# Dellintel98/smart-nanogrid-gym

Measured on AMD Instinct MI355X. Metric: env-steps/sec (whole node) at N=65,536 envs × 10 chargers, 24-step day, higher is better.
Workload: dtype f64; 1 GPU; 65536 envs/GPU x 10 chargers x 24-step day, b-pv bounded sparse 1h, GPU-RNG reset + 24 fused steps per bench step (hipGraph); envs_per_gpu=65536, chargers=10, step_unit=one simulated day of every env, days_per_graph_replay=11, parallelism=env-sharded x1

## Files before the change

include/sng.h:

```cpp
#ifndef SNG_H
#define SNG_H

#include <stddef.h>
#include <stdint.h>

#ifdef __cplusplus
extern "C" {
#endif

#define SNG_ABI_VERSION 10

typedef enum SngStatus {
    SNG_OK = 0,
    SNG_ERR_INVALID_ARGUMENT = -1,
    SNG_ERR_UNSUPPORTED = -2,
    SNG_ERR_HIP = -3,
    SNG_ERR_STATE = -4,
    SNG_ERR_OUT_OF_MEMORY = -5
} SngStatus;

typedef enum SngPenaltyMode {
    SNG_PENALTY_NONE = 0,
    SNG_PENALTY_ON_DEPARTURE = 1,
    SNG_PENALTY_SPARSE = 2,
// ... 130 lines not shown

int sng_state_size(const SngEnv *env, int with_episode_return, size_t *bytes);
int sng_get_state(SngEnv *env, void *host_buf, size_t bytes, const double *episode_return, void *stream);
int sng_set_state(SngEnv *env, const void *host_buf, size_t bytes, double *episode_return, void *stream);

int sng_get_scenario(SngEnv *env, int64_t first, int64_t count, int32_t max_vehicles, double *soc,
                     double *occupancy, double *capacity, double *requested_soc, int32_t *arrivals,
                     int32_t *departures, int32_t *n_vehicles, double *pv_ratio, void *stream);

int sng_get_tables(const SngEnv *env, double *irr, double *irr_max, double *pv_power, double *price,
                   double *price_max, int32_t *n);

#define SNG_GRAPH_RESET 1
#define SNG_GRAPH_STEP_NODES 2
#define SNG_GRAPH_TRAJECTORY 4
int sng_graph_create(SngEnv *env, const float *actions, float *obs, double *reward, uint8_t *done,
                     const SngInfo *info, int flags, int32_t days, double *day_returns, SngGraph **out);
int sng_graph_launch(SngGraph *graph, void *stream);
int sng_graph_step_nodes(const SngGraph *graph);
int sng_time_step_kernels(SngEnv *env, const float *actions, float *obs, double *reward, uint8_t *done,
                          const SngInfo *info, int32_t days, float *ms, float *reset_ms, void *stream);
void sng_graph_destroy(SngGraph *graph);

int sng_host_generate_scenarios(const SngConfig *cfg, int64_t num_envs, uint64_t seed, int32_t episodes,
                                double *soc, double *occupancy, double *capacity, double *requested_soc,
                                int32_t *arrivals, int32_t *departures, int32_t max_vehicles,
                                double *pv_ratio);

int32_t sng_host_threads(void);

int sng_get_day_counter(SngEnv *env, uint64_t *out, void *stream);

int sng_bandwidth_probe(int device, int64_t read_bytes, int64_t write_bytes, int32_t reps, float *dispatch_us,
                        float *back_to_back_us, void *stream);
// ... 15 lines not shown
```

smart-nanogrid-gym_amd/csrc/sng_api.cpp:

```cpp
#include <atomic>
#include <condition_variable>
#include <cstring>
#include <mutex>
#include <thread>

#include "sng_env.h"
#include "sng_host_day.h"
#include "sng_host_pool.h"
#include "sng_mt.h"

using namespace sng;

namespace sng {

thread_local std::string g_create_error;

int ensure_req(SngEnv *env) {
    if (!env->ds.req) HIP_TRY(env, hipMalloc(&env->ds.req, env->timeline() * sizeof(double)));
    return SNG_OK;
}

int await_prepare(SngEnv *env, hipStream_t st) {
    if (env->prep_launched) HIP_TRY(env, hipStreamWaitEvent(st, env->prep_done, 0));
    return SNG_OK;
}

int alloc_streams(SngEnv *env, RefStreams &r) {
    if (r.mt) return SNG_OK;
    HIP_TRY(env, hipMalloc(&r.mt, (size_t)env->E * 2 * kMtN * sizeof(uint32_t)));
    HIP_TRY(env, hipMalloc(&r.pos, (size_t)env->E * sizeof(int32_t)));
    return SNG_OK;
}

// ... 294 lines not shown
    *out = env;
    return SNG_OK;
}

void sng_destroy(SngEnv *env) {
    if (!env) return;
    DeviceScope scope(env->device);
    if (env->prep_stream) {
        (void)hipStreamSynchronize(env->prep_stream);
        (void)hipStreamDestroy(env->prep_stream);
        (void)hipEventDestroy(env->prep_done);
        (void)hipEventDestroy(env->day_drawn);
    }
    DeviceState &ds = env->ds;
    void *dev[] = {ds.soc, ds.bess, ds.bess0, ds.ratio, ds.pen0, ds.word, ds.aux, ds.req, ds.flags, ds.prof_key,
                   ds.episode, env->d_tables, env->rs.mt, env->rs.pos, env->ps.mt, env->ps.pos};
    for (void *x : dev)
        if (x) (void)hipFree(x);
    void *host[] = {env->h_word, env->h_aux, env->h_req, env->h_ratio, env->h_pen0};
    for (void *x : host)
        if (x) (void)hipHostFree(x);
    if (env->staging_done) (void)hipEventDestroy(env->staging_done);
    if (env->hio) (void)hipHostFree(env->hio);
    delete env;
}

int sng_get_dims(const SngEnv *env, SngDims *out) {
    if (!env || !out) return SNG_ERR_INVALID_ARGUMENT;
    out->obs_dim = env->p.obs_dim;
    out->act_dim = env->p.act_dim;
    out->timesteps = env->p.T;
// ... 383 lines not shown
```

smart-nanogrid-gym_amd/csrc/sng_env.h:

```cpp
#pragma once
#include <hip/hip_runtime.h>

#include <string>
#include <vector>

#include "sng.h"
#include "sng_device_scope.h"
#include "sng_host_tables.h"
#include "sng_launch.h"
#include "sng_layout.h"
#include "sng_state_format.h"

struct SngEnv {
    SngConfig cfg{};
    sng::Params p{};
    sng::HostTables tables;
    sng::Tables host_tab{};
    uint64_t cfg_hash = 0;
    std::vector<double> irradiance;
    int device = 0;
    int64_t E = 0;
    uint64_t seed = 0;
    int t = -1;
    bool day_finished = false;
    sng::DaySpans spans{0, 0, 0, sng::kSlots};
    int gen_mode = -1;
    bool gen_loaded = false;
    uint64_t replays = 0;
    sng::DeviceState ds{};
    sng::Tables *d_tables = nullptr;
    uint32_t *h_word = nullptr;
    double *h_aux = nullptr, *h_req = nullptr, *h_ratio = nullptr, *h_pen0 = nullptr;
    hipEvent_t staging_done = nullptr;
    sng::RefStreams rs{};
    bool np_seeded = false;
    hipStream_t prep_stream = nullptr;
    hipEvent_t prep_done = nullptr, day_drawn = nullptr;
    bool prep_launched = false;

    bool prepared = false;
    sng::RefStreams ps{};
    bool py_seeded = false;
    char *hio = nullptr, *hio_dev = nullptr;
    size_t hio_bytes = 0;
    std::string err;

    size_t timeline() const { return (size_t)p.T * p.n * (size_t)E; }
};

struct SngGraph {
    SngEnv *env = nullptr;
    bool with_reset = false;
    bool day_kernel = false;
    sng::DayKey key{};
    uint64_t seed = 0;
    int64_t env_offset = 0;
    hipGraph_t graph = nullptr;
    hipGraphExec_t exec = nullptr;
};

#pragma GCC visibility push(hidden)
namespace sng {

extern thread_local std::string g_create_error;

inline int fail(SngEnv *env, int code, const std::string &msg) {
    if (env) env->err = msg; else g_create_error = msg;
    return code;
// ... 53 lines not shown
    o.bess_power = i->battery_power_value;
    o.bess_calc_power = i->battery_calculated_power;
    o.nonexistent = i->nonexistent_vehicle_penalty;
    o.bess_initial = i->initial_battery_soc;
    o.flags = i->flags;
    o.episode_return = i->episode_return;
    o.charger_power = i->charger_power;
    o.vehicle_soc = i->vehicle_soc;
    o.flag_any = i->flag_summary;
    return o;
}

inline hipStream_t as_stream(void *s) { return (hipStream_t)s; }

int ensure_req(SngEnv *env);
int await_prepare(SngEnv *env, hipStream_t st);
int alloc_streams(SngEnv *env, RefStreams &r);
int ensure_np_streams(SngEnv *env, hipStream_t st);

}
#pragma GCC visibility pop
```

smart-nanogrid-gym_amd/csrc/sng_generate.h:

```cpp
#pragma once

namespace sng {

struct HashStream {
    uint32_t key, ctr;
    __device__ __forceinline__ uint32_t next() { return mix32(key + (ctr++) * 0x9e3779b9u); }
};

__device__ __forceinline__ double u32_unit(uint32_t x) { return (double)x * 0x1.0p-32; }

__device__ __forceinline__ int below(uint32_t x, int n) {
    return (int)(((uint64_t)x * (uint64_t)n) >> 32);
}

constexpr uint32_t kDomainRatio = 0x7a710000u;
constexpr uint32_t kDomainReplay = 0x7a720000u;

__device__ __forceinline__ double pv_ratio_draw(uint64_t seed, uint64_t ge, uint64_t day) {
    HashStream r2{stream_key(seed, ge, kDomainRatio, day), 0u};
    return (double)below(r2.next(), 181) / 100;
}

__device__ __forceinline__ double replay_ratio_draw(uint64_t seed, uint64_t ge, uint64_t replay) {
    HashStream r2{stream_key(seed, ge, kDomainReplay, replay), 0u};
// ... 167 lines not shown
    const uint32_t r = ((x1 & 0xffu) << 8) | (x2 & 0xffu);
    const uint32_t rc = r * 105u;
    d.cap = p.diff_caps ? 15u + (rc >> 16) : 40u;
    const uint32_t yd = (p.diff_caps ? rc : r) & 0xffffu;
    const int hi_c = d.ta + i10, hi_d = p.T + i1;
    const int high = hi_c < hi_d ? hi_c : hi_d;
    const int low = d.ta + i4;
    d.dep = (low >= high) ? low : low + (int)(__umul24(yd, (uint32_t)(high - low)) >> 16);
    d.req_draw = p.req_enabled ? rng.next() : 0u;
    return d;
}

constexpr int kObsParts = kGenBlock / kWave;
constexpr int kObsEnvs = kGenBlock / kObsParts;
constexpr int kObsBlocks = kGenBlock / kObsEnvs;
__device__ __forceinline__ void observe_day0(const Params &p, const DeviceState &s, uint64_t seed, int64_t E, int i4,
                                             int i10, int i1, uint64_t day, float *__restrict__ obs,
                                             double *__restrict__ ep_return, int vec_io, float *lds, int q) {
    const int n = p.n, O = p.obs_dim;
    const int tid = threadIdx.x, part = __builtin_amdgcn_readfirstlane(tid / kWave), le = tid % kWave;
    const int64_t e0 = (int64_t)blockIdx.x * kGenBlock + (int64_t)q * kObsEnvs;
    if (e0 >= E) return;
    const int nblk = (int)((E - e0) < kObsEnvs ? (E - e0) : kObsEnvs);
    const int64_t e = e0 + le;
    float *o_row = lds + le * O;
    if (le < nblk) {
        const uint64_t ge = (uint64_t)(e + p.env_offset);
        const uint64_t env_seed = p.seed + (uint64_t)p.env_offset + (uint64_t)e;
        if (p.noise && part == 0) {
            s.prof_key[2 * e] = stream_key(env_seed, 0, kDomainPV, day);
            s.prof_key[2 * e + 1] = stream_key(env_seed, 0, kDomainPrice, day);
        }
        if (part == 0) {
            const double ratio = pv_ratio_draw(seed, ge, day);
            s.ratio[e] = ratio;
            s.pen0[e] = 0.0;
            double fpv[4] = {1.0, 1.0, 1.0, 1.0}, fpr[4] = {1.0, 1.0, 1.0, 1.0};
            if (p.noise) {
#pragma unroll
                for (int k = 0; k < 4; ++k) {
                    if (p.pv_noise != 0.0) fpv[k] = profile_factor(env_seed, kDomainPV, day, k, p.pv_noise);
                    if (p.price_noise != 0.0) fpr[k] = profile_factor(env_seed, kDomainPrice, day, k, p.price_noise);
                }
            }
            write_obs_header(o_row, p, s.tables->irr_norm, s.tables->price_norm, ratio, fpv, fpr);
            if (p.bess) o_row[O - 1] = (float)s.bess[e];
            if (ep_return) ep_return[e] = 0.0;
        }
        const int k = p.pv ? 8 : 4;
        const uint32_t el8 = (uint32_t)e * 8u;
        for (int c0 = 2 * (part - 1); part > 0 && c0 < n; c0 += 2 * (kObsParts - 1)) {
            double soc0[2] = {0.0, 0.0};
#pragma unroll
            for (int i = 0; i < 2; ++i) {
                const int c = c0 + i;
                if (c >= n) break;
                GenStream rng{gen_key(seed, ge, (uint32_t)c, day), 0u};
                const VehicleDraw d = draw_vehicle(p, rng, 0, i4, i10, i1);
                const bool occ0 = d.ta == 0;
                soc0[i] = occ0 ? d.soc : 0.0;
                o_row[k + c] = (float)soc0[i];
                o_row[k + n + c] = departure_obs(pack_word(occ0, occ0, false, 0u, occ0 ? (uint32_t)d.dep : 0u));
            }
            const SocOff so = soc_off(c0, n, E, el8);
            if (c0 + 1 < n)
                bst2<kNT>(s.soc, so.v, soc0[0], soc0[1], so.s);
            else
                bst<kNT>(s.soc, so.v, soc0[0], so.s);
        }
    }
    __syncthreads();
    copy_out<kGenBlock>(obs + e0 * O, lds, nblk * O, vec_io != 0, tid);
}

constexpr int kGenRecPol = kNT;
__host__ __device__ constexpr int gen_part_lanes(int w) { return w == 3 ? 4 : w; }
__host__ __device__ constexpr int gen_rows(int n) { return 4 * (n / 4) + (n % 4 == 0 ? 0 : 4 * gen_part_lanes(n % 4) / 4); }
constexpr int kVehArrShift = 24;
constexpr uint32_t kVehRecMask = 0x3fff8u;
template <int TT, bool REQ>
__global__ __launch_bounds__(kGenBlock) void generate_kernel(Params p, DeviceState s, uint64_t seed, int64_t E,
                                                             int i4, int i10, int i1, float *__restrict__ obs,
                                                             double *__restrict__ ep_return, int vec_io) {
    extern __shared__ __attribute__((aligned(16))) float lds[];
    uint32_t *s_veh = reinterpret_cast<uint32_t *>(lds);
    uint32_t *s_car = s_veh + kDaySlots * kGenBlock;
    double *s_req = reinterpret_cast<double *>(s_car + kDaySlots * kGenBlock);
    const int tid = threadIdx.x;
    const int u = (int)blockIdx.y;
    const uint64_t day = *s.episode;
    if (u >= gen_rows(p.n)) {
        observe_day0(p, s, seed, E, i4, i10, i1, day, obs, ep_return, vec_io, lds, u - gen_rows(p.n));
        return;
    }
    const int full = 4 * (p.n / 4);
    const int q4 = u < full ? (u >> 2) * 4 : p.n & ~3;
    const int qw = p.n - q4 < 4 ? p.n - q4 : 4;
    const int lpe = u < full ? 4 : gen_part_lanes(qw);
    const int sub = u < full ? (u & 3) : u - full;
    const int c = q4 + tid % lpe;
    const int64_t e = (int64_t)blockIdx.x * kGenBlock + (int64_t)sub * (kGenBlock / lpe) + tid / lpe;
    if (e >= E || c >= p.n) return;
    const uint64_t ge = (uint64_t)(e + p.env_offset);
    GenStream rng{gen_key(seed, ge, (uint32_t)c, day), 0u};
    const int T = TT > 0 ? TT : p.T;
// ... 71 lines not shown
```

smart-nanogrid-gym_amd/csrc/sng_graph.cpp:

```cpp
#include <algorithm>

#include "sng_env.h"

using namespace sng;

extern "C" {

int sng_graph_create(SngEnv *env, const float *actions, float *obs, double *reward, uint8_t *done,
                     const SngInfo *info, int flags, int32_t days, double *day_returns, SngGraph **out) {
    const bool with_reset = (flags & SNG_GRAPH_RESET) != 0;
    if (!env || !actions || !obs || !reward || !done || !out) return fail(env, SNG_ERR_INVALID_ARGUMENT, "null argument");
    if (days < 1 || (days > 1 && !with_reset))
        return fail(env, SNG_ERR_INVALID_ARGUMENT, "days must be >= 1 (more than one needs SNG_GRAPH_RESET)");
    if (with_reset && !device_rng_ok(env))
        return fail(env, SNG_ERR_UNSUPPORTED, "device RNG needs time_interval <= 2h");
    ON_DEVICE_OF(env);
    if (env->p.req_enabled) SNG_TRY(ensure_req(env));
    hipStream_t cs;
    HIP_TRY(env, hipStreamCreateWithFlags(&cs, hipStreamNonBlocking));
    SngGraph *g = new SngGraph();
    g->env = env;
    g->with_reset = with_reset;
    g->key = with_reset ? DayKey::device_day(env->p) : DayKey::of(env->p);
    const Params p = with_day(env->p, g->key);
    g->seed = env->seed;
    g->env_offset = p.env_offset;
    const InfoPtrs ip = info_ptrs(info);
    const DaySpans &sp = env->spans;
    const int64_t E = env->E;
    const int A = p.act_dim;
    const int vec = (aligned16(actions) && aligned16(obs)) ? 1 : 0;
    const bool traj = (flags & SNG_GRAPH_TRAJECTORY) != 0;
    const size_t obs_block = (size_t)E * (size_t)p.obs_dim;
    const int64_t obs_step = traj ? (int64_t)obs_block : 0, out_step = traj ? E : 0;
    g->day_kernel = !(flags & SNG_GRAPH_STEP_NODES) && day_kernel_available(p, ip, traj) != 0;
    hipError_t e = hipStreamBeginCapture(cs, hipStreamCaptureModeThreadLocal);
    for (int d = 0; e == hipSuccess && d < days; ++d) {
        InfoPtrs ipd = ip;
        if (day_returns) ipd.episode_return = day_returns + (size_t)d * E;
        float *obs0 = obs + (traj ? (size_t)d * (size_t)(p.T + 1) * obs_block : 0);
        float *obs_d = obs0 + obs_step;
        double *reward_d = reward + (traj ? (size_t)d * (size_t)p.T * (size_t)E : 0);
        uint8_t *done_d = done + (traj ? (size_t)d * (size_t)p.T * (size_t)E : 0);
        if (with_reset) {
            e = launch_generate(p, env->ds, env->seed, E, sp.i4, sp.i10, sp.i1, obs0, ipd.episode_return,
                                (vec && aligned16(obs0)) ? 1 : 0, cs);
        }
        if (g->day_kernel) {
            if (e == hipSuccess)
                e = launch_day(p, env->ds, ipd, actions, obs_d, reward_d, done_d, E, 0, p.T,
                               (vec && aligned16(obs_d)) ? 1 : 0, cs, obs_step, out_step);
            continue;
        }
        for (int t = 0; e == hipSuccess && t < p.T; ++t) {
            float *obs_t = obs_d + (size_t)t * (size_t)obs_step;
            e = launch_step(p, env->ds, ipd, env->host_tab, actions + (size_t)t * E * A, obs_t,
                            reward_d + (size_t)t * (size_t)out_step, done_d + (size_t)t * (size_t)out_step, E, t,
                            (vec && aligned16(obs_t)) ? 1 : 0, cs);
        }
    }
    hipGraph_t graph = nullptr;
    hipError_t e2 = hipStreamEndCapture(cs, &graph);
    if (e == hipSuccess) e = e2;
    if (e == hipSuccess) e = hipGraphInstantiate(&g->exec, graph, nullptr, nullptr, 0);
    (void)hipStreamDestroy(cs);
    if (e != hipSuccess) {
        if (graph) (void)hipGraphDestroy(graph);
        delete g;
        return hip_fail(env, e, "graph capture");
    }
    g->graph = graph;
    *out = g;
    return SNG_OK;
}

int sng_graph_launch(SngGraph *g, void *stream) {
    if (!g) return SNG_ERR_INVALID_ARGUMENT;
    SngEnv *env = g->env;
    if (!g->with_reset) {
        if (!(g->key == DayKey::of(env->p)))
// ... 6 lines not shown
        return fail(env, SNG_ERR_STATE, "seed or env offset changed since the graph was captured: recapture it");
    ON_DEVICE_OF(env);
    if (g->with_reset) HIP_TRY(env, count_unstepped_device_day(env, as_stream(stream)));
    HIP_TRY(env, hipGraphLaunch(g->exec, as_stream(stream)));
    if (g->with_reset) {
        load_day(env, g->key);
        generated_day_loaded(env, SNG_RNG_DEVICE);
    }
    days_ran(env);
    return SNG_OK;
}

int sng_graph_step_nodes(const SngGraph *g) {
    if (!g) return -1;
    return g->day_kernel ? 1 : g->env->p.T;
}

void sng_graph_destroy(SngGraph *g) {
    if (!g) return;
    DeviceScope scope(g->env->device);
    if (g->exec) (void)hipGraphExecDestroy(g->exec);
    if (g->graph) (void)hipGraphDestroy(g->graph);
    delete g;
}

int sng_time_step_kernels(SngEnv *env, const float *actions, float *obs, double *reward, uint8_t *done,
                          const SngInfo *info, int32_t days, float *ms, float *reset_ms, void *stream) {
    if (!env || !actions || !obs || !reward || !done || days < 1)
        return fail(env, SNG_ERR_INVALID_ARGUMENT, "null argument");
    if (!device_rng_ok(env)) return fail(env, SNG_ERR_UNSUPPORTED, "device RNG needs time_interval <= 2h");
// ... 79 lines not shown
```

smart-nanogrid-gym_amd/csrc/sng_kernels.hip:

```cpp
#include <hip/hip_ext.h>
#include <hip/hip_runtime.h>
#include <stdint.h>

#include "sng.h"
#include "sng_launch.h"
#include "sng_layout.h"
#include "sng_step_plan.h"

#include "sng_dev_util.h"
#include "sng_dev_sums.h"
#include "sng_dev_env.h"
#include "sng_step_lean.h"
#include "sng_step_wide.h"
#include "sng_step_day.h"
#include "sng_step_general.h"
#include "sng_generate.h"

namespace sng {

__global__ __launch_bounds__(256) void probe_copy_kernel(const float4 *__restrict__ in, float4 *__restrict__ out,
                                                         int64_t nr, int64_t nw) {
    const int64_t i = (int64_t)blockIdx.x * 256 + threadIdx.x;
    typedef float v4f __attribute__((ext_vector_type(4)));
    v4f v = {0.f, 0.f, 0.f, 0.f};
// ... 146 lines not shown
    else return nullptr;
}
template <int NC>
static StepLaunch day_lean_launch(const StepPlan &pl, int64_t E, DayLeanKernel &kern) {
    kern = day_lean_entry<NC, false, false>();
    if (pl.pk && pl.req) kern = day_lean_entry<NC, true, true>();
    else if (pl.pk) kern = day_lean_entry<NC, true, false>();
    else if (pl.req) kern = day_lean_entry<NC, false, true>();
    return {nullptr, nullptr, blocks_for(E, kLeanBlock), dim3(kLeanBlock), LeanLds<NC>::BYTES};
}

int day_kernel_available(const Params &p, const InfoPtrs &info, bool trajectory) {
    return day_kernel_of(step_plan(p, info_diag(info)), trajectory) != DAY_NONE ? 1 : 0;
}

hipError_t launch_day(const Params &p, const DeviceState &s, const InfoPtrs &info, const float *act, float *obs,
                      double *reward, uint8_t *done, int64_t E, int t0, int nt, int vec_io, hipStream_t stream,
                      int64_t obs_step, int64_t out_step) {
    const StepPlan pl = step_plan(p, info_diag(info));
    const DayFamily fam = day_kernel_of(pl, obs_step != 0 || out_step != 0);
    if (fam == DAY_NONE) return hipErrorNotSupported;
    if (t0 < 0 || nt < 1 || t0 + nt > p.T) return hipErrorInvalidValue;
    if (fam == DAY_WIDE) {
        DayKernel kern = nullptr;
        const StepLaunch l = day_launch<10>(pl, E, kern);
        return launch_kernel(kern, l.grid, l.block, l.lds, stream, nullptr, nullptr, act, obs, reward, done, E, t0, nt,
                             vec_io, p, s, info);
    }
    DayLeanKernel kern = nullptr;
    StepLaunch l;
// ... 18 lines not shown
hipError_t launch_observe0(const Params &p, const DeviceState &s, float *obs, double *ep_return, int64_t E,
                           int vec_io, hipStream_t stream, int mode, int64_t replay, const RefStreams *ps, int py) {
    const RefStreams no_streams{nullptr, nullptr};
    const RefStreams &pss = (py && ps) ? *ps : no_streams;
    if (!ps) py = 0;
    const bool big = (size_t)round4(256 * p.obs_dim) * 4 <= 64 * 1024;
    const int envs = big ? 256 : kWave;
    auto kern = big ? (p.packed ? observe0_kernel<256, true> : observe0_kernel<256, false>)
                    : (p.packed ? observe0_kernel<kWave, true> : observe0_kernel<kWave, false>);
    return launch_kernel(kern, blocks_for(E, envs), dim3(envs), (size_t)round4(envs * p.obs_dim) * 4, stream, nullptr,
                         nullptr, p, s, obs, ep_return, E, vec_io, mode, replay, pss, py);
}

hipError_t launch_generate(const Params &p, const DeviceState &s, uint64_t seed, int64_t E, int i4, int i10, int i1,
                           float *obs, double *ep_return, int vec_io, hipStream_t stream, hipEvent_t ev_start,
                           hipEvent_t ev_stop) {
    const size_t veh = generate_lds_bytes(p.req_enabled != 0), tile = (size_t)round4(kObsEnvs * p.obs_dim) * 4;
    const bool fused = tile <= 32 * 1024;
    const dim3 grid((unsigned)((E + kGenBlock - 1) / kGenBlock), (unsigned)(gen_rows(p.n) + (fused ? kObsBlocks : 0))),
        block(kGenBlock);
    const size_t lds = (fused && tile > veh) ? tile : veh;
    const bool req = p.req_enabled != 0;
    auto kern = p.T == 24 ? (req ? generate_kernel<24, true> : generate_kernel<24, false>)
                : (p.T == 96 && !req) ? generate_kernel<96, false>
                : (req ? generate_kernel<0, true> : generate_kernel<0, false>);
    if (fused && ev_start && ev_stop)
        return launch_kernel(kern, grid, block, lds, stream, ev_start, ev_stop, p, s, seed, E, i4, i10, i1, obs,
                             ep_return, vec_io);
    if (ev_start) (void)hipEventRecord(ev_start, stream);
    hipError_t e = launch_kernel(kern, grid, block, lds, stream, nullptr, nullptr, p, s, seed, E, i4, i10, i1, obs,
                                 ep_return, vec_io);
    if (!fused) {
        if (e == hipSuccess) e = launch_profiles(p, s, E, stream);
        if (e == hipSuccess) e = launch_observe0(p, s, obs, ep_return, E, vec_io, stream, OBS0_DEVICE, -1);
    }
    if (e == hipSuccess && ev_stop) e = hipEventRecord(ev_stop, stream);
    return e;
}

}

#include "sng_ref_day.h"

namespace sng {

static int ref_day2_envs(int64_t E) {
// ... 40 lines not shown
    if (prepare) {
        hipError_t e = launch_mt_prepare(rs, E, stream);
        if (e != hipSuccess) return e;
    }
    const bool req = p.req_stream != 0;
    if (p.T == 24) {
        if (req) launch_ref_day2<24, true>(p, s, rs, E, i4, i10, i1, stream);
        else launch_ref_day2<24, false>(p, s, rs, E, i4, i10, i1, stream);
    } else {
        if (req) launch_ref_day2<0, true>(p, s, rs, E, i4, i10, i1, stream);
        else launch_ref_day2<0, false>(p, s, rs, E, i4, i10, i1, stream);
    }
    return hipGetLastError();
}

__global__ void bump_day_kernel(DeviceState s) { *s.episode += 1; }

hipError_t launch_bump_day(const DeviceState &s, hipStream_t stream) {
    hipLaunchKernelGGL(bump_day_kernel, dim3(1), dim3(1), 0, stream, s);
    return hipGetLastError();
}

hipError_t launch_profiles(const Params &p, const DeviceState &s, int64_t E, hipStream_t stream) {
    if (!p.noise) return hipSuccess;
    const dim3 grid((unsigned)((E + 255) / 256)), block(256);
    hipLaunchKernelGGL(profile_kernel, grid, block, 0, stream, p, s, E);
    return hipGetLastError();
}

}
```

smart-nanogrid-gym_amd/csrc/sng_launch.h:

```cpp
#pragma once
#include <hip/hip_runtime.h>

#include "sng_layout.h"

namespace sng {

hipError_t launch_step(const Params &p, const DeviceState &s, const InfoPtrs &info, const Tables &tab,
                       const float *act, float *obs, double *reward, uint8_t *done, int64_t E, int t, int vec_io,
                       hipStream_t stream, hipEvent_t ev_start = nullptr, hipEvent_t ev_stop = nullptr);
int day_kernel_available(const Params &p, const InfoPtrs &info, bool trajectory = false);
hipError_t launch_day(const Params &p, const DeviceState &s, const InfoPtrs &info, const float *act, float *obs,
                      double *reward, uint8_t *done, int64_t E, int t0, int nt, int vec_io, hipStream_t stream,
                      int64_t obs_step = 0, int64_t out_step = 0);
hipError_t launch_observe0(const Params &p, const DeviceState &s, float *obs, double *ep_return, int64_t E,
                           int vec_io, hipStream_t stream, int mode, int64_t replay, const RefStreams *ps = nullptr,
                           int py = 0);
hipError_t launch_generate(const Params &p, const DeviceState &s, uint64_t seed, int64_t E, int i4, int i10, int i1,
                           float *obs, double *ep_return, int vec_io, hipStream_t stream,
                           hipEvent_t ev_start = nullptr, hipEvent_t ev_stop = nullptr);
hipError_t launch_profiles(const Params &p, const DeviceState &s, int64_t E, hipStream_t stream);
hipError_t launch_bump_day(const DeviceState &s, hipStream_t stream);
hipError_t launch_probe_copy(const void *in, void *out, int64_t nr, int64_t nw, hipStream_t stream, hipEvent_t a,
                             hipEvent_t b);
hipError_t launch_ref_seed(const RefStreams &rs, uint64_t seed0, int64_t E, hipStream_t stream);
hipError_t launch_mt_prepare(const RefStreams &rs, int64_t E, hipStream_t stream);
hipError_t launch_ref_day(const Params &p, const DeviceState &s, const RefStreams &rs, int64_t E, int i4, int i10,
                          int i1, bool prepare, hipStream_t stream);
int step_lanes_supported(int n, int lanes);
int step_kernel_name(const Params &p, const InfoPtrs &info, char *buf, int len);

}
```

smart-nanogrid-gym_amd/csrc/sng_step_plan.h:

```cpp
#pragma once
#include <stdio.h>

#include "sng_layout.h"

namespace sng {

struct StationSize {
    int n;
    bool lean, wide, lanes;
};
constexpr StationSize kStationSizes[] = {
    {1, true, false, false}, {2, true, false, true},  {4, true, false, true},  {8, true, false, true},
    {10, true, true, true},  {16, true, false, true}, {50, false, true, true},
};
inline const StationSize *station_size(int n) {
    for (const StationSize &s : kStationSizes)
        if (s.n == n) return &s;
    return nullptr;
}

inline bool station_lanes_supported(int n, int lanes) {
    const StationSize *s = station_size(n);
    return lanes == 1 || ((lanes == 2 || lanes == 4) && s && s->lanes);
}
// ... 25 lines not shown
        pl.family = STEP_WIDE;
        pl.lanes = kWideLanes;
    }
    return pl;
}

enum DayFamily : int { DAY_NONE, DAY_WIDE, DAY_LEAN };
constexpr bool day_lean_compiled(int nc, bool pk, bool req) { return !(nc == 1 && pk && req); }
inline DayFamily day_kernel_of(const StepPlan &pl, bool trajectory) {
    const StationSize *sz = station_size(pl.nc);
    if (pl.diag || !sz) return DAY_NONE;
    if (pl.family == STEP_LEAN && sz->lean) return day_lean_compiled(pl.nc, pl.pk, pl.req) ? DAY_LEAN : DAY_NONE;
    if (pl.family == STEP_WIDE && pl.pk && pl.lanes == kWideLanes && pl.nc == 10 && !trajectory) return DAY_WIDE;
    return DAY_NONE;
}
inline int day_plan_name(const StepPlan &pl, bool trajectory, char *buf, int len) {
    auto b = [](bool v) { return v ? "true" : "false"; };
    switch (day_kernel_of(pl, trajectory)) {
        case DAY_LEAN:
            return snprintf(buf, (size_t)len, "void sng::day_lean_kernel<%d, %s, %s>", pl.nc, b(pl.pk), b(pl.req));
        case DAY_WIDE:
            return snprintf(buf, (size_t)len, "void sng::day_wide_kernel<%d, %d, %s, %s>", pl.nc, pl.lanes, b(pl.req),
                            b(pl.noise));
        default: break;
    }
    return snprintf(buf, (size_t)len, "%s", "");
}

inline int step_plan_name(const StepPlan &pl, char *buf, int len) {
    auto b = [](bool v) { return v ? "true" : "false"; };
// ... 11 lines not shown
```

smart-nanogrid-gym_amd/smart_nanogrid_gym/_native.py:

```python
import ctypes
import os

try:
    import torch
except Exception:
    torch = None

PKG_DIR = os.path.dirname(os.path.abspath(__file__))
LIB_PATH = os.environ.get("SNG_LIBRARY", os.path.join(os.path.dirname(PKG_DIR), "lib", "libsng.so"))
DATA_DIR = os.path.join(PKG_DIR, "data")
IRRADIANCE_FILE = os.path.join(DATA_DIR, "solar_irradiance_1min.f64")

ABI_VERSION = 10
SNG_OK = 0
RNG_REFERENCE = 0
RNG_DEVICE = 1
GRAPH_RESET = 1
GRAPH_STEP_NODES = 2
GRAPH_TRAJECTORY = 4
FLAG_NEGATIVE_DEMAND = 0x1
FLAG_CHARGING_MODE = 0x2
FLAG_BESS_SOC_ABOVE_1 = 0x4
FLAG_V2X_BREAKPOINT = 0x8
FLAG_SUMMARY_WORDS = 1024
COMM_ID_BYTES = 128

c_double_p = ctypes.POINTER(ctypes.c_double)
c_float_p = ctypes.POINTER(ctypes.c_float)
c_int32_p = ctypes.POINTER(ctypes.c_int32)
c_uint32_p = ctypes.POINTER(ctypes.c_uint32)


class SngConfig(ctypes.Structure):
    _fields_ = [
# ... 85 lines not shown
    "sng_get_pv_ratio": (ctypes.c_int, [_H, c_double_p, _S]),
    "sng_get_vehicle_soc": (ctypes.c_int, [_H, c_double_p, _S]),
    "sng_set_vehicle_soc": (ctypes.c_int, [_H, c_double_p, _S]),
    "sng_state_size": (ctypes.c_int, [_H, ctypes.c_int, ctypes.POINTER(ctypes.c_size_t)]),
    "sng_get_state": (ctypes.c_int, [_H, ctypes.c_void_p, ctypes.c_size_t, ctypes.c_void_p, _S]),
    "sng_set_state": (ctypes.c_int, [_H, ctypes.c_void_p, ctypes.c_size_t, ctypes.c_void_p, _S]),
    "sng_get_scenario": (ctypes.c_int, [_H, ctypes.c_int64, ctypes.c_int64, ctypes.c_int32, c_double_p, c_double_p,
                                        c_double_p, c_double_p, c_int32_p, c_int32_p, c_int32_p, c_double_p, _S]),
    "sng_get_tables": (ctypes.c_int, [_H, c_double_p, c_double_p, c_double_p, c_double_p, c_double_p,
                                      c_int32_p]),
    "sng_graph_create": (ctypes.c_int, [_H, ctypes.c_void_p, ctypes.c_void_p, ctypes.c_void_p,
                                        ctypes.c_void_p, ctypes.POINTER(SngInfo), ctypes.c_int, ctypes.c_int32,
                                        ctypes.c_void_p, ctypes.POINTER(ctypes.c_void_p)]),
    "sng_graph_launch": (ctypes.c_int, [ctypes.c_void_p, _S]),
    "sng_graph_step_nodes": (ctypes.c_int, [ctypes.c_void_p]),
    "sng_graph_destroy": (None, [ctypes.c_void_p]),
    "sng_time_step_kernels": (ctypes.c_int, [_H, ctypes.c_void_p, ctypes.c_void_p, ctypes.c_void_p,
                                             ctypes.c_void_p, ctypes.POINTER(SngInfo), ctypes.c_int32, c_float_p,
                                             c_float_p, _S]),
    "sng_host_generate_scenarios": (ctypes.c_int, [ctypes.POINTER(SngConfig), ctypes.c_int64, ctypes.c_uint64,
                                                   ctypes.c_int32, c_double_p, c_double_p, c_double_p, c_double_p,
                                                   c_int32_p, c_int32_p, ctypes.c_int32, c_double_p]),
    "sng_host_threads": (ctypes.c_int32, []),
    "sng_get_day_counter": (ctypes.c_int, [_H, ctypes.POINTER(ctypes.c_uint64), _S]),
    "sng_bandwidth_probe": (ctypes.c_int, [ctypes.c_int, ctypes.c_int64, ctypes.c_int64, ctypes.c_int32,
                                           ctypes.POINTER(ctypes.c_float), ctypes.POINTER(ctypes.c_float), _S]),
    "sng_comm_unique_id": (ctypes.c_int, [ctypes.c_char_p]),
    "sng_comm_create": (ctypes.c_int, [ctypes.c_int, ctypes.c_int, ctypes.c_int, ctypes.c_char_p,
                                       ctypes.POINTER(ctypes.c_void_p)]),
    "sng_allgather_returns": (ctypes.c_int, [ctypes.c_void_p, ctypes.c_void_p, ctypes.c_void_p, ctypes.c_int64, _S]),
# ... 47 lines not shown
```

smart-nanogrid-gym_amd/smart_nanogrid_gym/vec_env.py:

```python
import collections.abc
import ctypes
import itertools
import operator
import time
import warnings

import numpy as np

from . import _native
from ._native import check, lib
from .settings import (BESS_ABOVE_ONE, NEGATIVE_DEMAND, WRONG_CHARGING_MODE, WRONG_PENALTY_MODE, EnvSettings)
from .spaces import make_spaces

try:
    import torch
except Exception:
    torch = None

try:
    from stable_baselines3.common.vec_env import VecEnv as _VecEnvBase
except Exception:
    _VecEnvBase = object

SLOTS = 25
# ... 720 lines not shown
        irr = np.zeros(512)
        pv = np.zeros(512)
        price = np.zeros(512)
        mx = ctypes.c_double()
        pmx = ctypes.c_double()
        P = _native.c_double_p
        check(lib().sng_get_tables(self._h, irr.ctypes.data_as(P), ctypes.byref(mx), pv.ctypes.data_as(P),
                                   price.ctypes.data_as(P), ctypes.byref(pmx), ctypes.byref(n)), self._h)
        n_price = 2 * self.timesteps if self.settings.constants.get("extended_day") else 48
        return dict(irr=irr[:n.value], irr_max=mx.value, pv_power=pv[:n.value], price=price[:n_price],
                    price_max=pmx.value)


class EpisodeGraph:

    def __init__(self, venv, actions, with_reset=True, days=1, day_returns=None, step_nodes=False, trajectory=False):
        if with_reset:
            venv._apply_pending_seed()
        elif venv._seeds[0] is not None:
            raise ValueError("seed() waits for the next reset: reset before capturing a steps-only graph")
        self.venv = venv
        self.days = int(days)
        self.with_reset = bool(with_reset)
        self.trajectory = bool(trajectory)
        self.actions = actions.contiguous()
        self.day_returns = day_returns
        dr = None
        if day_returns is not None:
            if (tuple(day_returns.shape) != (self.days, venv.num_envs) or day_returns.dtype != torch.float64
                    or day_returns.device != venv.device or not day_returns.is_contiguous()):
                raise ValueError("day_returns must be a contiguous float64 device tensor [days, num_envs]")
# ... 2 lines not shown
        self.obs_traj = self.reward_traj = self.done_traj = None
        if self.trajectory:
            T, E = venv.timesteps, venv.num_envs
            self.obs_traj = obs = torch.zeros((self.days, T + 1, E, venv.obs_dim), dtype=torch.float32,
                                              device=venv.device)
            self.reward_traj = reward = torch.zeros((self.days, T, E), dtype=torch.float64, device=venv.device)
            self.done_traj = done = torch.zeros((self.days, T, E), dtype=torch.uint8, device=venv.device)
        g = ctypes.c_void_p()
        with torch.cuda.device(venv.device):
            check(lib().sng_graph_create(venv._h, ctypes.c_void_p(self.actions.data_ptr()),
                                         ctypes.c_void_p(obs.data_ptr()),
                                         ctypes.c_void_p(reward.data_ptr()),
                                         ctypes.c_void_p(done.data_ptr()), ctypes.byref(venv._info),
                                         (_native.GRAPH_RESET if with_reset else 0)
                                         | (_native.GRAPH_STEP_NODES if step_nodes else 0)
                                         | (_native.GRAPH_TRAJECTORY if self.trajectory else 0),
                                         self.days, dr, ctypes.byref(g)), venv._h)
        self._g = g

    @property
    def step_nodes_per_day(self):
        return int(lib().sng_graph_step_nodes(self._g))

    def launch(self, stream=None):
        s = _stream_handle(self.venv.device) if stream is None else ctypes.c_void_p(stream)
        if self.trajectory and not self.with_reset:
            if stream is None:
                self.obs_traj[0, 0].copy_(self.venv.obs_d)
            else:
                with torch.cuda.stream(torch.cuda.ExternalStream(stream, device=self.venv.device)):
                    self.obs_traj[0, 0].copy_(self.venv.obs_d)
        check(lib().sng_graph_launch(self._g, s), self.venv._h)

    def close(self):
        if getattr(self, "_g", None):
            lib().sng_graph_destroy(self._g)
            self._g = None
# ... 7 lines not shown
```

Before: 16.60 billion env-steps/s.

## Overlap next-day scenario generation with current-day stepping via double-buffered state

Within a multi-day captured graph, the reset generator for day d+1 now runs on a second stream into a shadow copy of per-day state while the day-d step kernel runs, with events enforcing ping-pong slot reuse. The generator skips writing observations and takes a day offset, and the day counter is bumped once at the end. The goal is to hide the reset kernel's latency behind the stepping kernel. In exchange it uses extra device memory, forces a larger generator LDS allocation that limits how many generator blocks fit alongside step blocks, and adds event dependencies between the two streams.

```diff
diff --git a/include/sng.h b/include/sng.h
--- a/include/sng.h
+++ b/include/sng.h
@@ -168,10 +168,13 @@
 #define SNG_GRAPH_RESET 1
 #define SNG_GRAPH_STEP_NODES 2
 #define SNG_GRAPH_TRAJECTORY 4
+#define SNG_GRAPH_SERIAL_RESET 8
+#define SNG_GRAPH_OVERLAPPED_RESET 16
 int sng_graph_create(SngEnv *env, const float *actions, float *obs, double *reward, uint8_t *done,
                      const SngInfo *info, int flags, int32_t days, double *day_returns, SngGraph **out);
 int sng_graph_launch(SngGraph *graph, void *stream);
 int sng_graph_step_nodes(const SngGraph *graph);
+int sng_graph_reset_overlapped(const SngGraph *graph);
 int sng_time_step_kernels(SngEnv *env, const float *actions, float *obs, double *reward, uint8_t *done,
                           const SngInfo *info, int32_t days, float *ms, float *reset_ms, void *stream);
 void sng_graph_destroy(SngGraph *graph);
diff --git a/smart-nanogrid-gym_amd/csrc/sng_api.cpp b/smart-nanogrid-gym_amd/csrc/sng_api.cpp
--- a/smart-nanogrid-gym_amd/csrc/sng_api.cpp
+++ b/smart-nanogrid-gym_amd/csrc/sng_api.cpp
@@ -17,6 +17,38 @@
 
 int ensure_req(SngEnv *env) {
     if (!env->ds.req) HIP_TRY(env, hipMalloc(&env->ds.req, env->timeline() * sizeof(double)));
+    return SNG_OK;
+}
+
+int ensure_shadow(SngEnv *env, DeviceState *out) {
+    DaySlot &sh = env->shadow;
+    const Params &p = env->p;
+    const size_t E = (size_t)env->E;
+    const size_t rec_bytes = (size_t)(p.T + 2) * (size_t)p.n * ((E + 255) / 256 * 256) * sizeof(uint16_t);
+    struct {
+        void **ptr;
+        size_t bytes;
+    } const arrays[] = {
+        {(void **)&sh.soc, E * p.n * sizeof(double)},
+        {(void **)&sh.ratio, E * sizeof(double)},
+        {(void **)&sh.pen0, E * sizeof(double)},
+        {(void **)&sh.aux, rec_bytes},
+        {(void **)&sh.day_return, E * sizeof(double)},
+        {(void **)&sh.req, env->ds.req ? env->timeline() * sizeof(double) : 0},
+        {(void **)&sh.prof_key, p.noise ? 2 * E * sizeof(uint32_t) : 0},
+    };
+    for (const auto &a : arrays) {
+        if (*a.ptr || !a.bytes) continue;
+        HIP_TRY(env, hipMalloc(a.ptr, a.bytes));
+        HIP_TRY(env, hipMemset(*a.ptr, 0, a.bytes));
+    }
+    *out = env->ds;
+    out->soc = sh.soc;
+    out->ratio = sh.ratio;
+    out->pen0 = sh.pen0;
+    out->aux = sh.aux;
+    out->req = sh.req;
+    out->prof_key = sh.prof_key;
     return SNG_OK;
 }
 
@@ -341,7 +373,9 @@
     }
     DeviceState &ds = env->ds;
     void *dev[] = {ds.soc, ds.bess, ds.bess0, ds.ratio, ds.pen0, ds.word, ds.aux, ds.req, ds.flags, ds.prof_key,
-                   ds.episode, env->d_tables, env->rs.mt, env->rs.pos, env->ps.mt, env->ps.pos};
+                   ds.episode, env->d_tables, env->rs.mt, env->rs.pos, env->ps.mt, env->ps.pos,
+                   env->shadow.soc, env->shadow.ratio, env->shadow.pen0, env->shadow.aux, env->shadow.req,
+                   env->shadow.prof_key, env->shadow.day_return};
     for (void *x : dev)
         if (x) (void)hipFree(x);
     void *host[] = {env->h_word, env->h_aux, env->h_req, env->h_ratio, env->h_pen0};
diff --git a/smart-nanogrid-gym_amd/csrc/sng_env.h b/smart-nanogrid-gym_amd/csrc/sng_env.h
--- a/smart-nanogrid-gym_amd/csrc/sng_env.h
+++ b/smart-nanogrid-gym_amd/csrc/sng_env.h
@@ -10,6 +10,12 @@
 #include "sng_launch.h"
 #include "sng_layout.h"
 #include "sng_state_format.h"
+
+struct DaySlot {
+    double *soc = nullptr, *ratio = nullptr, *pen0 = nullptr, *aux = nullptr, *req = nullptr;
+    uint32_t *prof_key = nullptr;
+    double *day_return = nullptr;
+};
 
 struct SngEnv {
     SngConfig cfg{};
@@ -28,6 +34,7 @@
     bool gen_loaded = false;
     uint64_t replays = 0;
     sng::DeviceState ds{};
+    DaySlot shadow{};
     sng::Tables *d_tables = nullptr;
     uint32_t *h_word = nullptr;
     double *h_aux = nullptr, *h_req = nullptr, *h_ratio = nullptr, *h_pen0 = nullptr;
@@ -52,6 +59,7 @@
     SngEnv *env = nullptr;
     bool with_reset = false;
     bool day_kernel = false;
+    bool overlapped = false;
     sng::DayKey key{};
     uint64_t seed = 0;
     int64_t env_offset = 0;
@@ -135,6 +143,7 @@
 inline hipStream_t as_stream(void *s) { return (hipStream_t)s; }
 
 int ensure_req(SngEnv *env);
+int ensure_shadow(SngEnv *env, DeviceState *out);
 int await_prepare(SngEnv *env, hipStream_t st);
 int alloc_streams(SngEnv *env, RefStreams &r);
 int ensure_np_streams(SngEnv *env, hipStream_t st);
diff --git a/smart-nanogrid-gym_amd/csrc/sng_generate.h b/smart-nanogrid-gym_amd/csrc/sng_generate.h
--- a/smart-nanogrid-gym_amd/csrc/sng_generate.h
+++ b/smart-nanogrid-gym_amd/csrc/sng_generate.h
@@ -205,6 +205,7 @@
 constexpr int kObsParts = kGenBlock / kWave;
 constexpr int kObsEnvs = kGenBlock / kObsParts;
 constexpr int kObsBlocks = kGenBlock / kObsEnvs;
+static_assert(kObsEnvs == kGenObsEnvs, "generator_fused (sng_step_plan.h) sizes the observation tile");
 __device__ __forceinline__ void observe_day0(const Params &p, const DeviceState &s, uint64_t seed, int64_t E, int i4,
                                              int i10, int i1, uint64_t day, float *__restrict__ obs,
                                              double *__restrict__ ep_return, int vec_io, float *lds, int q) {
@@ -234,8 +235,10 @@
                     if (p.price_noise != 0.0) fpr[k] = profile_factor(env_seed, kDomainPrice, day, k, p.price_noise);
                 }
             }
-            write_obs_header(o_row, p, s.tables->irr_norm, s.tables->price_norm, ratio, fpv, fpr);
-            if (p.bess) o_row[O - 1] = (float)s.bess[e];
+            if (obs) {
+                write_obs_header(o_row, p, s.tables->irr_norm, s.tables->price_norm, ratio, fpv, fpr);
+                if (p.bess) o_row[O - 1] = (float)s.bess[e];
+            }
             if (ep_return) ep_return[e] = 0.0;
         }
         const int k = p.pv ? 8 : 4;
@@ -250,8 +253,10 @@
                 const VehicleDraw d = draw_vehicle(p, rng, 0, i4, i10, i1);
                 const bool occ0 = d.ta == 0;
                 soc0[i] = occ0 ? d.soc : 0.0;
-                o_row[k + c] = (float)soc0[i];
-                o_row[k + n + c] = departure_obs(pack_word(occ0, occ0, false, 0u, occ0 ? (uint32_t)d.dep : 0u));
+                if (obs) {
+                    o_row[k + c] = (float)soc0[i];
+                    o_row[k + n + c] = departure_obs(pack_word(occ0, occ0, false, 0u, occ0 ? (uint32_t)d.dep : 0u));
+                }
             }
             const SocOff so = soc_off(c0, n, E, el8);
             if (c0 + 1 < n)
@@ -260,6 +265,7 @@
                 bst<kNT>(s.soc, so.v, soc0[0], so.s);
         }
     }
+    if (!obs) return;
     __syncthreads();
     copy_out<kGenBlock>(obs + e0 * O, lds, nblk * O, vec_io != 0, tid);
 }
@@ -272,14 +278,15 @@
 template <int TT, bool REQ>
 __global__ __launch_bounds__(kGenBlock) void generate_kernel(Params p, DeviceState s, uint64_t seed, int64_t E,
                                                              int i4, int i10, int i1, float *__restrict__ obs,
-                                                             double *__restrict__ ep_return, int vec_io) {
+                                                             double *__restrict__ ep_return, int vec_io,
+                                                             int day_delta) {
     extern __shared__ __attribute__((aligned(16))) float lds[];
     uint32_t *s_veh = reinterpret_cast<uint32_t *>(lds);
     uint32_t *s_car = s_veh + kDaySlots * kGenBlock;
     double *s_req = reinterpret_cast<double *>(s_car + kDaySlots * kGenBlock);
     const int tid = threadIdx.x;
     const int u = (int)blockIdx.y;
-    const uint64_t day = *s.episode;
+    const uint64_t day = *s.episode + (uint64_t)day_delta;
     if (u >= gen_rows(p.n)) {
         observe_day0(p, s, seed, E, i4, i10, i1, day, obs, ep_return, vec_io, lds, u - gen_rows(p.n));
         return;
diff --git a/smart-nanogrid-gym_amd/csrc/sng_graph.cpp b/smart-nanogrid-gym_amd/csrc/sng_graph.cpp
--- a/smart-nanogrid-gym_amd/csrc/sng_graph.cpp
+++ b/smart-nanogrid-gym_amd/csrc/sng_graph.cpp
@@ -34,36 +34,97 @@
     const size_t obs_block = (size_t)E * (size_t)p.obs_dim;
     const int64_t obs_step = traj ? (int64_t)obs_block : 0, out_step = traj ? E : 0;
     g->day_kernel = !(flags & SNG_GRAPH_STEP_NODES) && day_kernel_available(p, ip, traj) != 0;
-    hipError_t e = hipStreamBeginCapture(cs, hipStreamCaptureModeThreadLocal);
-    for (int d = 0; e == hipSuccess && d < days; ++d) {
+    size_t generator_lds = 0;
+    g->overlapped = with_reset && reset_graph_overlapped(p, ip, days, traj, (flags & SNG_GRAPH_SERIAL_RESET) != 0,
+                                                         (flags & SNG_GRAPH_OVERLAPPED_RESET) != 0, &generator_lds) != 0;
+    DeviceState slots[2] = {env->ds, env->ds};
+    hipStream_t gs = nullptr;
+    std::vector<hipEvent_t> generated, stepped;
+    hipError_t e = hipSuccess;
+    if (g->overlapped) {
+        if (int rc = ensure_shadow(env, &slots[1])) {
+            (void)hipStreamDestroy(cs);
+            delete g;
+            return rc;
+        }
+        generated.assign((size_t)days, nullptr);
+        stepped.assign((size_t)days, nullptr);
+        e = hipStreamCreateWithFlags(&gs, hipStreamNonBlocking);
+        for (int d = 0; d < days; ++d) {
+            if (e == hipSuccess) e = hipEventCreateWithFlags(&generated[(size_t)d], hipEventDisableTiming);
+            if (e == hipSuccess) e = hipEventCreateWithFlags(&stepped[(size_t)d], hipEventDisableTiming);
+        }
+    }
+    auto row = [&](int d, const DayShape &sh) {
         InfoPtrs ipd = ip;
         if (day_returns) ipd.episode_return = day_returns + (size_t)d * E;
+        else if (sh.slot && ip.episode_return) ipd.episode_return = env->shadow.day_return;
+        return ipd;
+    };
+    auto capture_generator = [&](int d) {
+        const DayShape sh = day_shape(true, days, d);
+        if (d >= 2) e = hipStreamWaitEvent(gs, stepped[(size_t)d - 2], 0);
+        if (e == hipSuccess)
+            e = launch_generate(p, slots[sh.slot], env->seed, E, sp.i4, sp.i10, sp.i1, nullptr, row(d, sh).episode_return,
+                                0, gs, nullptr, nullptr, sh.day_delta, generator_lds);
+        if (e == hipSuccess) e = hipEventRecord(generated[(size_t)d], gs);
+        if (e == hipSuccess && sh.bump_node) e = launch_bump_day(env->ds, gs, (uint64_t)sh.bump_node);
+    };
+    if (e == hipSuccess) e = hipStreamBeginCapture(cs, hipStreamCaptureModeThreadLocal);
+    const bool capturing = e == hipSuccess;
+    if (g->overlapped && e == hipSuccess) {
+        e = hipEventRecord(stepped[0], cs);
+        if (e == hipSuccess) e = hipStreamWaitEvent(gs, stepped[0], 0);
+        if (e == hipSuccess) capture_generator(0);
+    }
+    for (int d = 0; e == hipSuccess && d < days; ++d) {
+        const DayShape sh = day_shape(g->overlapped, days, d);
+        const InfoPtrs ipd = row(d, sh);
+        const DeviceState &ds = slots[sh.slot];
+        Params pd = p;
+        if (g->overlapped) pd.bump_day = sh.bump_day;
         float *obs0 = obs + (traj ? (size_t)d * (size_t)(p.T + 1) * obs_block : 0);
         float *obs_d = obs0 + obs_step;
         double *reward_d = reward + (traj ? (size_t)d * (size_t)p.T * (size_t)E : 0);
         uint8_t *done_d = done + (traj ? (size_t)d * (size_t)p.T * (size_t)E : 0);
-        if (with_reset) {
-            e = launch_generate(p, env->ds, env->seed, E, sp.i4, sp.i10, sp.i1, obs0, ipd.episode_return,
+        if (g->overlapped) {
+            e = hipStreamWaitEvent(cs, generated[(size_t)d], 0);
+        } else if (with_reset) {
+            e = launch_generate(p, ds, env->seed, E, sp.i4, sp.i10, sp.i1, obs0, ipd.episode_return,
                                 (vec && aligned16(obs0)) ? 1 : 0, cs);
         }
         if (g->day_kernel) {
             if (e == hipSuccess)
-                e = launch_day(p, env->ds, ipd, actions, obs_d, reward_d, done_d, E, 0, p.T,
+                e = launch_day(pd, ds, ipd, actions, obs_d, reward_d, done_d, E, 0, p.T,
                                (vec && aligned16(obs_d)) ? 1 : 0, cs, obs_step, out_step);
-            continue;
-        }
-        for (int t = 0; e == hipSuccess && t < p.T; ++t) {
-            float *obs_t = obs_d + (size_t)t * (size_t)obs_step;
-            e = launch_step(p, env->ds, ipd, env->host_tab, actions + (size_t)t * E * A, obs_t,
-                            reward_d + (size_t)t * (size_t)out_step, done_d + (size_t)t * (size_t)out_step, E, t,
-                            (vec && aligned16(obs_t)) ? 1 : 0, cs);
-        }
+        } else {
+            for (int t = 0; e == hipSuccess && t < p.T; ++t) {
+                float *obs_t = obs_d + (size_t)t * (size_t)obs_step;
+                e = launch_step(pd, ds, ipd, env->host_tab, actions + (size_t)t * E * A, obs_t,
+                                reward_d + (size_t)t * (size_t)out_step, done_d + (size_t)t * (size_t)out_step, E, t,
+                                (vec && aligned16(obs_t)) ? 1 : 0, cs);
+            }
+        }
+        if (g->overlapped) {
+            if (e == hipSuccess) e = hipEventRecord(stepped[(size_t)d], cs);
+            if (e == hipSuccess && d + 1 < days) capture_generator(d + 1);
+        }
+    }
+    if (g->overlapped && capturing) {
+        hipError_t ej = hipEventRecord(generated[0], gs);
+        if (ej == hipSuccess) ej = hipStreamWaitEvent(cs, generated[0], 0);
+        if (e == hipSuccess) e = ej;
     }
     hipGraph_t graph = nullptr;
-    hipError_t e2 = hipStreamEndCapture(cs, &graph);
+    hipError_t e2 = capturing ? hipStreamEndCapture(cs, &graph) : hipSuccess;
     if (e == hipSuccess) e = e2;
     if (e == hipSuccess) e = hipGraphInstantiate(&g->exec, graph, nullptr, nullptr, 0);
     (void)hipStreamDestroy(cs);
+    if (gs) (void)hipStreamDestroy(gs);
+    for (hipEvent_t x : generated)
+        if (x) (void)hipEventDestroy(x);
+    for (hipEvent_t x : stepped)
+        if (x) (void)hipEventDestroy(x);
     if (e != hipSuccess) {
         if (graph) (void)hipGraphDestroy(graph);
         delete g;
@@ -100,6 +161,11 @@
 int sng_graph_step_nodes(const SngGraph *g) {
     if (!g) return -1;
     return g->day_kernel ? 1 : g->env->p.T;
+}
+
+int sng_graph_reset_overlapped(const SngGraph *g) {
+    if (!g) return -1;
+    return g->overlapped ? 1 : 0;
 }
 
 void sng_graph_destroy(SngGraph *g) {
diff --git a/smart-nanogrid-gym_amd/csrc/sng_kernels.hip b/smart-nanogrid-gym_amd/csrc/sng_kernels.hip
--- a/smart-nanogrid-gym_amd/csrc/sng_kernels.hip
+++ b/smart-nanogrid-gym_amd/csrc/sng_kernels.hip
@@ -184,6 +184,14 @@
     return day_kernel_of(step_plan(p, info_diag(info)), trajectory) != DAY_NONE ? 1 : 0;
 }
 
+int reset_graph_overlapped(const Params &p, const InfoPtrs &info, int days, bool trajectory, bool serial, bool force,
+                           size_t *generator_lds) {
+    const StepPlan pl = step_plan(p, info_diag(info));
+    if (!reset_overlapped(pl, p, days, trajectory, serial, force)) return 0;
+    if (generator_lds) *generator_lds = overlapped_generator_lds(pl);
+    return 1;
+}
+
 hipError_t launch_day(const Params &p, const DeviceState &s, const InfoPtrs &info, const float *act, float *obs,
                       double *reward, uint8_t *done, int64_t E, int t0, int nt, int vec_io, hipStream_t stream,
                       int64_t obs_step, int64_t out_step) {
@@ -232,22 +240,24 @@
 
 hipError_t launch_generate(const Params &p, const DeviceState &s, uint64_t seed, int64_t E, int i4, int i10, int i1,
                            float *obs, double *ep_return, int vec_io, hipStream_t stream, hipEvent_t ev_start,
-                           hipEvent_t ev_stop) {
+                           hipEvent_t ev_stop, int day_delta, size_t min_lds) {
     const size_t veh = generate_lds_bytes(p.req_enabled != 0), tile = (size_t)round4(kObsEnvs * p.obs_dim) * 4;
-    const bool fused = tile <= 32 * 1024;
+    const bool fused = generator_fused(p);
+    if (!fused && (day_delta != 0 || !obs)) return hipErrorInvalidValue;
     const dim3 grid((unsigned)((E + kGenBlock - 1) / kGenBlock), (unsigned)(gen_rows(p.n) + (fused ? kObsBlocks : 0))),
         block(kGenBlock);
-    const size_t lds = (fused && tile > veh) ? tile : veh;
+    size_t lds = (fused && obs && tile > veh) ? tile : veh;
+    if (min_lds > lds) lds = min_lds;
     const bool req = p.req_enabled != 0;
     auto kern = p.T == 24 ? (req ? generate_kernel<24, true> : generate_kernel<24, false>)
                 : (p.T == 96 && !req) ? generate_kernel<96, false>
                 : (req ? generate_kernel<0, true> : generate_kernel<0, false>);
     if (fused && ev_start && ev_stop)
         return launch_kernel(kern, grid, block, lds, stream, ev_start, ev_stop, p, s, seed, E, i4, i10, i1, obs,
-                             ep_return, vec_io);
+                             ep_return, vec_io, day_delta);
     if (ev_start) (void)hipEventRecord(ev_start, stream);
     hipError_t e = launch_kernel(kern, grid, block, lds, stream, nullptr, nullptr, p, s, seed, E, i4, i10, i1, obs,
-                                 ep_return, vec_io);
+                                 ep_return, vec_io, day_delta);
     if (!fused) {
         if (e == hipSuccess) e = launch_profiles(p, s, E, stream);
         if (e == hipSuccess) e = launch_observe0(p, s, obs, ep_return, E, vec_io, stream, OBS0_DEVICE, -1);
@@ -318,10 +328,12 @@
     return hipGetLastError();
 }
 
-__global__ void bump_day_kernel(DeviceState s) { *s.episode += 1; }
-
-hipError_t launch_bump_day(const DeviceState &s, hipStream_t stream) {
-    hipLaunchKernelGGL(bump_day_kernel, dim3(1), dim3(1), 0, stream, s);
+__global__ void bump_day_kernel(DeviceState s, uint64_t amount) {
+    __hip_atomic_fetch_add(s.episode, amount, __ATOMIC_RELAXED, __HIP_MEMORY_SCOPE_AGENT);
+}
+
+hipError_t launch_bump_day(const DeviceState &s, hipStream_t stream, uint64_t amount) {
+    hipLaunchKernelGGL(bump_day_kernel, dim3(1), dim3(1), 0, stream, s, amount);
     return hipGetLastError();
 }
 
diff --git a/smart-nanogrid-gym_amd/csrc/sng_launch.h b/smart-nanogrid-gym_amd/csrc/sng_launch.h
--- a/smart-nanogrid-gym_amd/csrc/sng_launch.h
+++ b/smart-nanogrid-gym_amd/csrc/sng_launch.h
@@ -17,9 +17,12 @@
                            int py = 0);
 hipError_t launch_generate(const Params &p, const DeviceState &s, uint64_t seed, int64_t E, int i4, int i10, int i1,
                            float *obs, double *ep_return, int vec_io, hipStream_t stream,
-                           hipEvent_t ev_start = nullptr, hipEvent_t ev_stop = nullptr);
+                           hipEvent_t ev_start = nullptr, hipEvent_t ev_stop = nullptr, int day_delta = 0,
+                           size_t min_lds = 0);
+int reset_graph_overlapped(const Params &p, const InfoPtrs &info, int days, bool trajectory, bool serial, bool force,
+                           size_t *generator_lds);
 hipError_t launch_profiles(const Params &p, const DeviceState &s, int64_t E, hipStream_t stream);
-hipError_t launch_bump_day(const DeviceState &s, hipStream_t stream);
+hipError_t launch_bump_day(const DeviceState &s, hipStream_t stream, uint64_t amount = 1);
 hipError_t launch_probe_copy(const void *in, void *out, int64_t nr, int64_t nw, hipStream_t stream, hipEvent_t a,
                              hipEvent_t b);
 hipError_t launch_ref_seed(const RefStreams &rs, uint64_t seed0, int64_t E, hipStream_t stream);
diff --git a/smart-nanogrid-gym_amd/csrc/sng_step_plan.h b/smart-nanogrid-gym_amd/csrc/sng_step_plan.h
--- a/smart-nanogrid-gym_amd/csrc/sng_step_plan.h
+++ b/smart-nanogrid-gym_amd/csrc/sng_step_plan.h
@@ -63,6 +63,24 @@
     if (pl.family == STEP_WIDE && pl.pk && pl.lanes == kWideLanes && pl.nc == 10 && !trajectory) return DAY_WIDE;
     return DAY_NONE;
 }
+constexpr int kGenObsEnvs = 64;
+inline bool generator_fused(const Params &p) { return (size_t)((kGenObsEnvs * p.obs_dim + 3) & ~3) * 4 <= 32 * 1024; }
+
+inline bool reset_overlapped(const StepPlan &pl, const Params &p, int days, bool trajectory, bool serial,
+                             bool force = false) {
+    const bool faster = pl.family == STEP_WIDE && pl.nc == 10;
+    return days >= 2 && !trajectory && !serial && generator_fused(p) && (faster || force);
+}
+inline size_t overlapped_generator_lds(const StepPlan &pl) { return pl.family == STEP_WIDE ? 56u * 1024u : 0u; }
+struct DayShape {
+    int slot, day_delta, bump_day, bump_node;
+};
+inline DayShape day_shape(bool overlapped, int days, int d) {
+    if (!overlapped) return {0, 0, 1, 0};
+    const bool last = d == days - 1;
+    return {(days - 1 - d) & 1, d, last ? 1 : 0, last ? days - 1 : 0};
+}
+
 inline int day_plan_name(const StepPlan &pl, bool trajectory, char *buf, int len) {
     auto b = [](bool v) { return v ? "true" : "false"; };
     switch (day_kernel_of(pl, trajectory)) {
diff --git a/smart-nanogrid-gym_amd/smart_nanogrid_gym/_native.py b/smart-nanogrid-gym_amd/smart_nanogrid_gym/_native.py
--- a/smart-nanogrid-gym_amd/smart_nanogrid_gym/_native.py
+++ b/smart-nanogrid-gym_amd/smart_nanogrid_gym/_native.py
@@ -18,6 +18,8 @@
 GRAPH_RESET = 1
 GRAPH_STEP_NODES = 2
 GRAPH_TRAJECTORY = 4
+GRAPH_SERIAL_RESET = 8
+GRAPH_OVERLAPPED_RESET = 16
 FLAG_NEGATIVE_DEMAND = 0x1
 FLAG_CHARGING_MODE = 0x2
 FLAG_BESS_SOC_ABOVE_1 = 0x4
@@ -133,6 +135,7 @@
                                         ctypes.c_void_p, ctypes.POINTER(ctypes.c_void_p)]),
     "sng_graph_launch": (ctypes.c_int, [ctypes.c_void_p, _S]),
     "sng_graph_step_nodes": (ctypes.c_int, [ctypes.c_void_p]),
+    "sng_graph_reset_overlapped": (ctypes.c_int, [ctypes.c_void_p]),
     "sng_graph_destroy": (None, [ctypes.c_void_p]),
     "sng_time_step_kernels": (ctypes.c_int, [_H, ctypes.c_void_p, ctypes.c_void_p, ctypes.c_void_p,
                                              ctypes.c_void_p, ctypes.POINTER(SngInfo), ctypes.c_int32, c_float_p,
diff --git a/smart-nanogrid-gym_amd/smart_nanogrid_gym/vec_env.py b/smart-nanogrid-gym_amd/smart_nanogrid_gym/vec_env.py
--- a/smart-nanogrid-gym_amd/smart_nanogrid_gym/vec_env.py
+++ b/smart-nanogrid-gym_amd/smart_nanogrid_gym/vec_env.py
@@ -758,7 +758,8 @@
 
 class EpisodeGraph:
 
-    def __init__(self, venv, actions, with_reset=True, days=1, day_returns=None, step_nodes=False, trajectory=False):
+    def __init__(self, venv, actions, with_reset=True, days=1, day_returns=None, step_nodes=False, trajectory=False,
+                 serial_reset=False, overlapped_reset=False):
         if with_reset:
             venv._apply_pending_seed()
         elif venv._seeds[0] is not None:
@@ -791,13 +792,19 @@
                                          ctypes.c_void_p(done.data_ptr()), ctypes.byref(venv._info),
                                          (_native.GRAPH_RESET if with_reset else 0)
                                          | (_native.GRAPH_STEP_NODES if step_nodes else 0)
-                                         | (_native.GRAPH_TRAJECTORY if self.trajectory else 0),
+                                         | (_native.GRAPH_TRAJECTORY if self.trajectory else 0)
+                                         | (_native.GRAPH_SERIAL_RESET if serial_reset else 0)
+                                         | (_native.GRAPH_OVERLAPPED_RESET if overlapped_reset else 0),
                                          self.days, dr, ctypes.byref(g)), venv._h)
         self._g = g
 
     @property
     def step_nodes_per_day(self):
         return int(lib().sng_graph_step_nodes(self._g))
+
+    @property
+    def reset_overlapped(self):
+        return bool(lib().sng_graph_reset_overlapped(self._g))
 
     def launch(self, stream=None):
         s = _stream_handle(self.venv.device) if stream is None else ctypes.c_void_p(stream)
```

New measurement: 17.78 billion env-steps/s, median of 6. 7.1% higher.
